# jdhuang-csm/hybrid-drt

Hardware: AMD Instinct MI355X
Metric: DRT fits/sec (256 freq x 512 tau, batched) (higher is better)
Workload: dtype f64

## Files before the change

### hybrid-drt_amd/csrc/gram.hip

```cpp
#include "common.hpp"

namespace hipdrt {

typedef double v4d __attribute__((ext_vector_type(4)));

static constexpr int GT = 64;
static constexpr int GK = 16;
static constexpr int GLD = 80;


template <bool DOP, bool ROWP>
__global__ __launch_bounds__(256, 5) void gram_kernel(int m, int n, const double* __restrict__ A, int lda,
                                                   const double* __restrict__ w, GramL2 g, double* __restrict__ P,
                                                   int ldp, long long p_stride, const int* __restrict__ active,
                                                   int ntile, double* __restrict__ Ppk, long long ppk_stride, int nchp,
                                                   long long a_stride) {
    const int b = blockIdx.y;
    if (active && !active[b]) return;
    A += (size_t)b * a_stride;
    int t = blockIdx.x, ti = 0;
    while (t >= ti + 1) { t -= ti + 1; ++ti; }
    const int tj = t;
    const int i0 = ti * GT, j0 = tj * GT;
    const bool diag = (ti == tj);

    __shared__ double sI[GK * GLD];
    __shared__ double sJ[GK * GLD];

    const int tid = threadIdx.x, lane = tid & 63, wv = tid >> 6;
    const int wi = (wv >> 1) * 32, wj = (wv & 1) * 32;
    const double* wb = w + (size_t)b * m;

    v4d acc[2][2];
#pragma unroll
    for (int a = 0; a < 2; ++a)
#pragma unroll
        for (int c = 0; c < 2; ++c) acc[a][c] = (v4d){0.0, 0.0, 0.0, 0.0};

    const int sk = tid >> 4, sc = (tid & 15) * 4;
    const bool vec2 = ((lda | n) & 1) == 0;
    double vi[4], vj[4], wkr = 0.0;
    auto fetch = [&](int k0) {
        const int k = k0 + sk;
#pragma unroll
        for (int e = 0; e < 4; ++e) { vi[e] = 0.0; vj[e] = 0.0; }
        wkr = 0.0;
        if (k < m) {
            wkr = wb[k];
            const double* row = A + (size_t)k * lda;
            if (vec2) {
#pragma unroll
                for (int e = 0; e < 4; e += 2) {
                    const int ci = i0 + sc + e, cj = j0 + sc + e;
                    if (ci < n) { const double2 t = *reinterpret_cast<const double2*>(row + ci); vi[e] = t.x; vi[e + 1] = t.y; }
                    if (!diag && cj < n) { const double2 t = *reinterpret_cast<const double2*>(row + cj); vj[e] = t.x; vj[e + 1] = t.y; }
                }
            } else {
#pragma unroll
                for (int e = 0; e < 4; ++e) {
                    const int ci = i0 + sc + e, cj = j0 + sc + e;
                    if (ci < n) vi[e] = row[ci];
                    if (!diag && cj < n) vj[e] = row[cj];
                }
            }
        }
    };
    const int nt16 = (n + 15) >> 4;
    const int tr0 = __builtin_amdgcn_readfirstlane((i0 + wi) >> 4), tc0 = __builtin_amdgcn_readfirstlane((j0 + wj) >> 4);
    const bool need00 = tr0 < nt16 && tc0 < nt16 && tr0 >= tc0;
    const bool need01 = tr0 < nt16 && tc0 + 1 < nt16 && tr0 >= tc0 + 1;
    const bool need10 = tr0 + 1 < nt16 && tc0 < nt16 && tr0 + 1 >= tc0;
    const bool need11 = tr0 + 1 < nt16 && tc0 + 1 < nt16 && tr0 + 1 >= tc0 + 1;
    fetch(0);
    for (int k0 = 0; k0 < m; k0 += GK) {
        __syncthreads();
        *reinterpret_cast<double2*>(&sI[sk * GLD + sc]) = make_double2(wkr * vi[0], wkr * vi[1]);
        *reinterpret_cast<double2*>(&sI[sk * GLD + sc + 2]) = make_double2(wkr * vi[2], wkr * vi[3]);
        if (!diag) {
            *reinterpret_cast<double2*>(&sJ[sk * GLD + sc]) = make_double2(wkr * vj[0], wkr * vj[1]);
            *reinterpret_cast<double2*>(&sJ[sk * GLD + sc + 2]) = make_double2(wkr * vj[2], wkr * vj[3]);
        }
        __syncthreads();
        if (k0 + GK < m) fetch(k0 + GK);
        const double* sj = diag ? sI : sJ;
#pragma unroll
        for (int kk = 0; kk < GK; kk += 4) {
            const int kr = kk + (lane >> 4);
            double a0 = sI[kr * GLD + wi + (lane & 15)];
            double a1 = sI[kr * GLD + wi + 16 + (lane & 15)];
            double b0 = sj[kr * GLD + wj + (lane & 15)];
            double b1 = sj[kr * GLD + wj + 16 + (lane & 15)];
            if (need00) acc[0][0] = __builtin_amdgcn_mfma_f64_16x16x4f64(b0, a0, acc[0][0], 0, 0, 0);
            if (need01) acc[0][1] = __builtin_amdgcn_mfma_f64_16x16x4f64(b1, a0, acc[0][1], 0, 0, 0);
            if (need10) acc[1][0] = __builtin_amdgcn_mfma_f64_16x16x4f64(b0, a1, acc[1][0], 0, 0, 0);
            if (need11) acc[1][1] = __builtin_amdgcn_mfma_f64_16x16x4f64(b1, a1, acc[1][1], 0, 0, 0);
        }
    }

    double (*sqI)[GT] = reinterpret_cast<double (*)[GT]>(sI);
    double (*sqJ)[GT] = reinterpret_cast<double (*)[GT]>(sJ);
    constexpr int TW = 2 * GT;
    double (*tw)[TW] = reinterpret_cast<double (*)[TW]>(sI + 3 * GT);
    const int dbase = i0 - j0 - (GT - 1);
    double fac[3] = {0, 0, 0};
    const bool l2on = g.s && !(!DOP && g.toep && g.toep_maxd >= 0 && (j0 >= g.ns || g.spec_zero) && i0 >= g.ns && dbase > g.toep_maxd);
    if (l2on) {
#pragma unroll
        for (int k = 0; k < 3; ++k) fac[k] = g.dfac[k] * (g.use_rho ? g.rho[(size_t)b * 3 + k] : 1.0);
        __syncthreads();
        const double* sb_ = g.s + (size_t)b * 3 * n;
        for (int e = tid; e < 3 * GT; e += 256) {
            const int k = e / GT, c = e % GT;
            sqI[k][c] = (i0 + c < n) ? sqrt(sb_[k * n + i0 + c]) : 0.0;
            sqJ[k][c] = (j0 + c < n) ? sqrt(sb_[k * n + j0 + c]) : 0.0;
        }
        if (g.toep) {
            const int nd = n - g.ns;
            for (int e = tid; e < 3 * TW; e += 256) {
                const int k = e / TW, sl = e % TW;
                int dd = dbase + sl;
                dd = dd < 0 ? -dd : dd;
                tw[k][sl] = (g.dfac[k] > 0.0 && dd < nd) ? g.mk[k][(size_t)g.ns * g.ldm + g.ns + dd] * fac[k] : 0.0;
            }
        }
        __syncthreads();
    }
    double* Pb = (ROWP && P) ? P + (size_t)b * p_stride : nullptr;
    double dfac2[3] = {0, 0, 0};
    if (l2on) {
        if (DOP) {
#pragma unroll
            for (int k = 0; k < 3; ++k) dfac2[k] = g.dop_dfac[k] * (g.use_rho ? g.dop_rho[(size_t)b * 3 + k] : 1.0);
        }
    }
    const int dop_lo = DOP ? g.dop_start : 0, dop_hi = DOP ? g.dop_start + g.dop_size : 0;
    double* Pk = Ppk ? Ppk + (size_t)b * ppk_stride : nullptr;
#pragma unroll
    for (int a = 0; a < 2; ++a)
#pragma unroll
        for (int c = 0; c < 2; ++c) {
            double vals[4];
#pragma unroll
            for (int r = 0; r < 4; ++r) {
                const int i = i0 + wi + a * 16 + (lane & 15);
                const int j = j0 + wj + c * 16 + (lane >> 4) + 4 * r;
                double v = 0.0;
                if (i < n && j < n) {
                    v = acc[a][c][r];
                    if (l2on) {
                        double l2 = 0.0;
#pragma unroll
                        for (int k = 0; k < 3; ++k) {
                            if (g.dfac[k] > 0.0) {
                                double mv;
                                if (g.toep && i >= g.ns && j >= g.ns) {
                                    mv = tw[k][(i - j) - dbase];
                                } else {
                                    mv = g.sym ? g.mk[k][(size_t)j * g.ldm + i] : g.mk[k][(size_t)i * g.ldm + j];
                                    if (i >= g.ns && j >= g.ns) mv *= fac[k];
                                    else if (DOP && i >= dop_lo && i < dop_hi && j >= dop_lo && j < dop_hi) mv *= dfac2[k];
                                }
                                l2 += (sqI[k][i - i0] * mv) * sqJ[k][j - j0];
                            }
                        }
                        v += l2;
                    } else if (!g.s && g.l2) {
                        v += g.l2[(size_t)b * g.l2_stride + (size_t)i * g.ldl2 + j];
                    }
                    if (ROWP && Pb && !(diag && j > i)) {
                        Pb[(size_t)i * ldp + j] = v;
                        if (i != j) Pb[(size_t)j * ldp + i] = v;
                    }
                }
                vals[r] = v;
            }
            if (Pk) {
                const int tr = ((i0 + wi) >> 4) + a, tc = ((j0 + wj) >> 4) + c;
                if (tr < nchp && tc < nchp && tr >= tc) {
                    double2* tile = reinterpret_cast<double2*>(Pk + ((size_t)tr * nchp + tc) * 256);
                    const int fo = (lane & 15) * 4 + (lane >> 4);
                    tile[fo] = make_double2(vals[0], vals[1]);
                    tile[64 + fo] = make_double2(vals[2], vals[3]);
                }
            }
        }
}

__global__ __launch_bounds__(64) void pack_p_kernel(int n, const double* __restrict__ P, int ldp, long long p_stride,
                                                    double* __restrict__ Ppk, long long ppk_stride, int nchp) {
    int t = blockIdx.x, tr = 0;
    while (t >= tr + 1) { t -= tr + 1; ++tr; }
    const int tc = t, b = blockIdx.y, lane = threadIdx.x;
    const double* Pb = P + (size_t)b * p_stride;
    double vals[4];
#pragma unroll
    for (int r = 0; r < 4; ++r) {
        const int i = tr * 16 + (lane & 15), j = tc * 16 + (lane >> 4) + 4 * r;
        double v = 0.0;
        if (i < n && j < n) v = (i >= j) ? Pb[(size_t)i * ldp + j] : Pb[(size_t)j * ldp + i];
        vals[r] = v;
    }
    double2* tile = reinterpret_cast<double2*>(Ppk + (size_t)b * ppk_stride + ((size_t)tr * nchp + tc) * 256);
    const int fo = (lane & 15) * 4 + (lane >> 4);
    tile[fo] = make_double2(vals[0], vals[1]);
    tile[64 + fo] = make_double2(vals[2], vals[3]);
}

__global__ __launch_bounds__(256) void qvec_kernel(int m, int n, const double* __restrict__ A, int lda,
                                                   const double* __restrict__ w, const double* __restrict__ y,
                                                   const double* __restrict__ l1, double l1_scalar,
                                                   double* __restrict__ q, const int* __restrict__ active,
                                                   long long a_stride) {
    const int b = blockIdx.y;
    if (active && !active[b]) return;
    A += (size_t)b * a_stride;
    __shared__ double sw[256], swy[256];
    const int i = blockIdx.x * 256 + threadIdx.x;
    const double* wb = w + (size_t)b * m;
    const double* yb = y + (size_t)b * m;
    double acc = 0.0;
    for (int k0 = 0; k0 < m; k0 += 256) {
        __syncthreads();
        const int kk = k0 + threadIdx.x;
        if (kk < m) { const double wk = wb[kk]; sw[threadIdx.x] = wk; swy[threadIdx.x] = wk * yb[kk]; }
        __syncthreads();
        const int lim = (m - k0) < 256 ? (m - k0) : 256;
        if (i < n) {
            for (int k = 0; k < lim; ++k) acc += (sw[k] * A[(size_t)(k0 + k) * lda + i]) * swy[k];
        }
    }
    if (i < n) q[(size_t)b * n + i] = -acc + (l1 ? l1[i] : l1_scalar);
}

__global__ __launch_bounds__(64) void pack_rows_kernel(int nrow, int ncol, int col_offset, const double* __restrict__ M,
                                                       int ldm, double* __restrict__ tiles, int nchp) {
    const int tr = blockIdx.y, tc = blockIdx.x, lane = threadIdx.x;
    double vals[4];
#pragma unroll
    for (int r = 0; r < 4; ++r) {
        const int i = tr * 16 + (lane & 15), j = tc * 16 + (lane >> 4) + 4 * r - col_offset;
        vals[r] = (i < nrow && j >= 0 && j < ncol) ? M[(size_t)i * ldm + j] : 0.0;
    }
    double2* tile = reinterpret_cast<double2*>(tiles + ((size_t)tr * nchp + tc) * 256);
    const int fo = (lane & 15) * 4 + (lane >> 4);
    tile[fo] = make_double2(vals[0], vals[1]);
    tile[64 + fo] = make_double2(vals[2], vals[3]);
}

void launch_pack_rows(hipStream_t st, int nrow, int ncol, int col_offset, const double* M, int ldm, int ntile_rows,
                      double* tiles, int nchp) {
    hipLaunchKernelGGL(pack_rows_kernel, dim3(nchp, ntile_rows), dim3(64), 0, st, nrow, ncol, col_offset, M, ldm, tiles,
                       nchp);
}

__global__ __launch_bounds__(256) void rows_outer_kernel(const double* __restrict__ Y, int nch, int ncol, int nrow, double scale,
                                                         double* __restrict__ out, int ld) {
    const int ti = blockIdx.y, tj = blockIdx.x;
    if (tj > ti) return;
    __shared__ double A[256], Bt[256];
    const int t = threadIdx.x, i = t >> 4, j = t & 15;
    auto at = [](int r, int k) { return 2 * ((k >> 3) * 64 + r * 4 + (k & 3)) + ((k >> 2) & 1); };
    double acc = 0.0;
    for (int c = 0; c < ncol; ++c) {
        A[t] = Y[((size_t)ti * nch + c) * 256 + t];
        Bt[t] = Y[((size_t)tj * nch + c) * 256 + t];
        __syncthreads();
#pragma unroll
        for (int k = 0; k < 16; ++k) acc += A[at(i, k)] * Bt[at(j, k)];
        __syncthreads();
    }
    const int r = ti * 16 + i, cc = tj * 16 + j;
    if (r < nrow && cc < nrow) {
        out[(size_t)r * ld + cc] = acc * scale;
        out[(size_t)cc * ld + r] = acc * scale;
    }
}

void launch_rows_outer(hipStream_t st, const double* Y, int nch, int ncol, int nex, int nrow, double scale, double* out, int ld) {
    hipLaunchKernelGGL(rows_outer_kernel, dim3(nex, nex), dim3(256), 0, st, Y, nch, ncol, nrow, scale, out, ld);
}

void launch_pack_p(hipStream_t st, int B, int n, const double* P, int ldp, long long p_stride, double* Ppk,
                   long long ppk_stride, int nchp) {
    const int nt = (n + 15) / 16;
    hipLaunchKernelGGL(pack_p_kernel, dim3(nt * (nt + 1) / 2, B), dim3(64), 0, st, n, P, ldp, p_stride, Ppk, ppk_stride,
                       nchp);
}

void launch_gram_l2(hipStream_t st, int B, int m, int n, const double* A, int lda, const double* w, const GramL2& g,
                    double* P, int ldp, long long p_stride, const int* active, double* Ppk, long long ppk_stride,
                    int nchp, long long a_stride) {
    const int nt = (n + GT - 1) / GT;
    const int ntile = nt * (nt + 1) / 2;
    const bool dop = g.s && g.dop_size > 0;
#define HIPDRT_GRAM(D, R) hipLaunchKernelGGL((gram_kernel<D, R>), dim3(ntile, B), dim3(256), 0, st, m, n, A, lda, w, g, P, ldp, \
                                             p_stride, active, ntile, Ppk, ppk_stride, nchp, a_stride)
    if (P) { if (dop) HIPDRT_GRAM(true, true); else HIPDRT_GRAM(false, true); }
    else { if (dop) HIPDRT_GRAM(true, false); else HIPDRT_GRAM(false, false); }
#undef HIPDRT_GRAM
}

void launch_qvec(hipStream_t st, int B, int m, int n, const double* A, int lda, const double* w, const double* y,
                 const double* l1, double l1_scalar, double* q, const int* active, long long a_stride) {
    if (a_stride == 0 && (size_t)m * n < ((size_t)1 << 20)) {
        launch_qvec_batched(st, B, m, n, A, lda, w, y, l1, l1_scalar, q, active);
        return;
    }
    hipLaunchKernelGGL(qvec_kernel, dim3((n + 255) / 256, B), dim3(256), 0, st, m, n, A, lda, w, y, l1, l1_scalar, q,
                       active, a_stride);
}

void launch_weighted_gram(hipStream_t st, int B, int m, int n, const double* A, int lda, const double* w,
                          const double* b, const double* l2, long long l2_stride, int ldl2, const double* l1,
                          double* P, int ldp, long long p_stride, double* q, const int* active) {
    GramL2 g{};
    g.l2 = l2; g.l2_stride = l2_stride; g.ldl2 = ldl2; g.s = nullptr;
    launch_gram_l2(st, B, m, n, A, lda, w, g, P, ldp, p_stride, active);
    launch_qvec(st, B, m, n, A, lda, w, b, l1, 0.0, q, active);
}

}
```

Measured before the change: 2649.

## Redistribute diagonal-tile MFMA work across waves and fold trailing 16-strip

Diagonal 64x64 Gram tiles now spread their ten lower-triangle 16x16 subtiles round-robin over the four waves. Before, waves owning upper-triangle blocks sat idle. When the number of 16-column chunks is 1 mod 4, the leftover 16-wide strip is folded into the diagonal tiles instead of getting its own row of 64-wide tiles, which cuts the tile count. The change adds templated per-turn code paths, extra shared-memory staging for the strip and its L2 weights, and explicit zeroing of padded packed tiles, so code size and complexity grow.

Result: faster. 2700 (median of 6 runs) (+1.9%).

```diff
diff --git a/hybrid-drt_amd/csrc/gram.hip b/hybrid-drt_amd/csrc/gram.hip
--- a/hybrid-drt_amd/csrc/gram.hip
+++ b/hybrid-drt_amd/csrc/gram.hip
@@ -1,4 +1,5 @@
 #include "common.hpp"
+#include <type_traits>
 
 namespace hipdrt {
 
@@ -8,6 +9,29 @@
 static constexpr int GK = 16;
 static constexpr int GLD = 80;
 
+
+__host__ __device__ inline bool gram_strip_folds(int n) { const int nt16 = (n + 15) >> 4; return (nt16 & 3) == 1 && nt16 > 1; }
+
+struct GramSub { int r, c; };
+__host__ __device__ constexpr GramSub gram_diag_sub(int e) {
+    const int r = e >= 10 ? 4 : e >= 6 ? 3 : e >= 3 ? 2 : e >= 1 ? 1 : 0;
+    return GramSub{r, e >= 14 ? 4 : e >= 10 ? e - 10 : e - r * (r + 1) / 2};
+}
+
+template <int TURN>
+__device__ __forceinline__ void gram_diag_slab(const double* sl, v4d (&acc)[4], int needm) {
+#pragma unroll
+    for (int kk = 0; kk < GK; kk += 4) {
+        double x[5];
+#pragma unroll
+        for (int c = 0; c < 5; ++c) x[c] = sl[kk * GLD + c * 16];
+#pragma unroll
+        for (int s = 0; s < 4; ++s) {
+            const GramSub sub = gram_diag_sub(TURN + 4 * s);
+            if (needm & (1 << s)) acc[s] = __builtin_amdgcn_mfma_f64_16x16x4f64(x[sub.c], x[sub.r], acc[s], 0, 0, 0);
+        }
+    }
+}
 
 template <bool DOP, bool ROWP>
 __global__ __launch_bounds__(256, 5) void gram_kernel(int m, int n, const double* __restrict__ A, int lda,
@@ -23,24 +47,41 @@
     const int tj = t;
     const int i0 = ti * GT, j0 = tj * GT;
     const bool diag = (ti == tj);
+    const int nt16 = (n + 15) >> 4;
+    const bool strip = diag && gram_strip_folds(n);
+    const int s0 = (nt16 - 1) * 16;
+    const bool last = strip && i0 + GT == s0;
 
     __shared__ double sI[GK * GLD];
     __shared__ double sJ[GK * GLD];
 
-    const int tid = threadIdx.x, lane = tid & 63, wv = tid >> 6;
-    const int wi = (wv >> 1) * 32, wj = (wv & 1) * 32;
+    const int tid = threadIdx.x, lane = tid & 63, wv = __builtin_amdgcn_readfirstlane(tid >> 6);
     const double* wb = w + (size_t)b * m;
-
-    v4d acc[2][2];
-#pragma unroll
-    for (int a = 0; a < 2; ++a)
-#pragma unroll
-        for (int c = 0; c < 2; ++c) acc[a][c] = (v4d){0.0, 0.0, 0.0, 0.0};
+    double* Pk = Ppk ? Ppk + (size_t)b * ppk_stride : nullptr;
+
+    int nown = 0, needm = 0;
+    const int turn = (wv + 2 * (ti & 1)) & 3;
+    if (diag) {
+        const int rows_all = (Pk && nchp > nt16 ? nchp : nt16) - 4 * ti, rows_data = nt16 - 4 * ti;
+        const int nr = rows_all < 4 ? rows_all : 4, nd = rows_data < 4 ? rows_data : 4;
+        nown = nr * (nr + 1) / 2 + (strip ? 4 : 0) + (last ? 1 : 0);
+        const int nneed = strip ? nown : nd * (nd + 1) / 2;
+#pragma unroll
+        for (int s = 0; s < 4; ++s) needm |= (turn + 4 * s < nneed) << s;
+    }
+    const int qr = 4 * ti + 2 * (wv >> 1), qc = 4 * tj + 2 * (wv & 1);
+    const bool need00 = qr < nt16 && qc < nt16, need01 = qr < nt16 && qc + 1 < nt16;
+    const bool need10 = qr + 1 < nt16 && qc < nt16, need11 = qr + 1 < nt16 && qc + 1 < nt16;
+
+    v4d acc[4];
+#pragma unroll
+    for (int s = 0; s < 4; ++s) acc[s] = (v4d){0.0, 0.0, 0.0, 0.0};
 
     const int sk = tid >> 4, sc = (tid & 15) * 4;
     const bool vec2 = ((lda | n) & 1) == 0;
     double vi[4], vj[4], wkr = 0.0;
-    auto fetch = [&](int k0) {
+    auto fetch = [&](auto DIAG, int k0) {
+        constexpr bool D = decltype(DIAG)::value;
         const int k = k0 + sk;
 #pragma unroll
         for (int e = 0; e < 4; ++e) { vi[e] = 0.0; vj[e] = 0.0; }
@@ -53,57 +94,73 @@
                 for (int e = 0; e < 4; e += 2) {
                     const int ci = i0 + sc + e, cj = j0 + sc + e;
                     if (ci < n) { const double2 t = *reinterpret_cast<const double2*>(row + ci); vi[e] = t.x; vi[e + 1] = t.y; }
-                    if (!diag && cj < n) { const double2 t = *reinterpret_cast<const double2*>(row + cj); vj[e] = t.x; vj[e + 1] = t.y; }
+                    if (!D && cj < n) { const double2 t = *reinterpret_cast<const double2*>(row + cj); vj[e] = t.x; vj[e + 1] = t.y; }
                 }
             } else {
 #pragma unroll
                 for (int e = 0; e < 4; ++e) {
                     const int ci = i0 + sc + e, cj = j0 + sc + e;
                     if (ci < n) vi[e] = row[ci];
-                    if (!diag && cj < n) vj[e] = row[cj];
+                    if (!D && cj < n) vj[e] = row[cj];
                 }
             }
+            if (D && strip && s0 + (tid & 15) < n) vj[0] = row[s0 + (tid & 15)];
         }
     };
-    const int nt16 = (n + 15) >> 4;
-    const int tr0 = __builtin_amdgcn_readfirstlane((i0 + wi) >> 4), tc0 = __builtin_amdgcn_readfirstlane((j0 + wj) >> 4);
-    const bool need00 = tr0 < nt16 && tc0 < nt16 && tr0 >= tc0;
-    const bool need01 = tr0 < nt16 && tc0 + 1 < nt16 && tr0 >= tc0 + 1;
-    const bool need10 = tr0 + 1 < nt16 && tc0 < nt16 && tr0 + 1 >= tc0;
-    const bool need11 = tr0 + 1 < nt16 && tc0 + 1 < nt16 && tr0 + 1 >= tc0 + 1;
-    fetch(0);
-    for (int k0 = 0; k0 < m; k0 += GK) {
-        __syncthreads();
-        *reinterpret_cast<double2*>(&sI[sk * GLD + sc]) = make_double2(wkr * vi[0], wkr * vi[1]);
-        *reinterpret_cast<double2*>(&sI[sk * GLD + sc + 2]) = make_double2(wkr * vi[2], wkr * vi[3]);
-        if (!diag) {
-            *reinterpret_cast<double2*>(&sJ[sk * GLD + sc]) = make_double2(wkr * vj[0], wkr * vj[1]);
-            *reinterpret_cast<double2*>(&sJ[sk * GLD + sc + 2]) = make_double2(wkr * vj[2], wkr * vj[3]);
-        }
-        __syncthreads();
-        if (k0 + GK < m) fetch(k0 + GK);
-        const double* sj = diag ? sI : sJ;
-#pragma unroll
-        for (int kk = 0; kk < GK; kk += 4) {
-            const int kr = kk + (lane >> 4);
-            double a0 = sI[kr * GLD + wi + (lane & 15)];
-            double a1 = sI[kr * GLD + wi + 16 + (lane & 15)];
-            double b0 = sj[kr * GLD + wj + (lane & 15)];
-            double b1 = sj[kr * GLD + wj + 16 + (lane & 15)];
-            if (need00) acc[0][0] = __builtin_amdgcn_mfma_f64_16x16x4f64(b0, a0, acc[0][0], 0, 0, 0);
-            if (need01) acc[0][1] = __builtin_amdgcn_mfma_f64_16x16x4f64(b1, a0, acc[0][1], 0, 0, 0);
-            if (need10) acc[1][0] = __builtin_amdgcn_mfma_f64_16x16x4f64(b0, a1, acc[1][0], 0, 0, 0);
-            if (need11) acc[1][1] = __builtin_amdgcn_mfma_f64_16x16x4f64(b1, a1, acc[1][1], 0, 0, 0);
-        }
-    }
-
-    double (*sqI)[GT] = reinterpret_cast<double (*)[GT]>(sI);
-    double (*sqJ)[GT] = reinterpret_cast<double (*)[GT]>(sJ);
+    auto kloop = [&](auto DIAG, auto TURN) {
+        constexpr bool D = decltype(DIAG)::value;
+        fetch(DIAG, 0);
+        for (int k0 = 0; k0 < m; k0 += GK) {
+            __syncthreads();
+            *reinterpret_cast<double2*>(&sI[sk * GLD + sc]) = make_double2(wkr * vi[0], wkr * vi[1]);
+            *reinterpret_cast<double2*>(&sI[sk * GLD + sc + 2]) = make_double2(wkr * vi[2], wkr * vi[3]);
+            if (!D) {
+                *reinterpret_cast<double2*>(&sJ[sk * GLD + sc]) = make_double2(wkr * vj[0], wkr * vj[1]);
+                *reinterpret_cast<double2*>(&sJ[sk * GLD + sc + 2]) = make_double2(wkr * vj[2], wkr * vj[3]);
+            } else if (strip) {
+                sI[sk * GLD + GT + (tid & 15)] = wkr * vj[0];
+            }
+            __syncthreads();
+            if (k0 + GK < m) fetch(DIAG, k0 + GK);
+            if (!D) {
+                const int wi = (wv >> 1) * 32, wj = (wv & 1) * 32;
+#pragma unroll
+                for (int kk = 0; kk < GK; kk += 4) {
+                    const int kr = kk + (lane >> 4);
+                    double a0 = sI[kr * GLD + wi + (lane & 15)];
+                    double a1 = sI[kr * GLD + wi + 16 + (lane & 15)];
+                    double b0 = sJ[kr * GLD + wj + (lane & 15)];
+                    double b1 = sJ[kr * GLD + wj + 16 + (lane & 15)];
+                    if (need00) acc[0] = __builtin_amdgcn_mfma_f64_16x16x4f64(b0, a0, acc[0], 0, 0, 0);
+                    if (need01) acc[1] = __builtin_amdgcn_mfma_f64_16x16x4f64(b1, a0, acc[1], 0, 0, 0);
+                    if (need10) acc[2] = __builtin_amdgcn_mfma_f64_16x16x4f64(b0, a1, acc[2], 0, 0, 0);
+                    if (need11) acc[3] = __builtin_amdgcn_mfma_f64_16x16x4f64(b1, a1, acc[3], 0, 0, 0);
+                }
+            } else {
+                const double* sl = sI + (lane >> 4) * GLD + (lane & 15);
+                gram_diag_slab<decltype(TURN)::value>(sl, acc, needm);
+            }
+        }
+    };
+    if (!diag) kloop(std::false_type{}, std::integral_constant<int, 0>{});
+    else if (turn == 0) kloop(std::true_type{}, std::integral_constant<int, 0>{});
+    else if (turn == 1) kloop(std::true_type{}, std::integral_constant<int, 1>{});
+    else if (turn == 2) kloop(std::true_type{}, std::integral_constant<int, 2>{});
+    else kloop(std::true_type{}, std::integral_constant<int, 3>{});
+
+    double* sqI = sI;
+    double* sqJ = sJ;
     constexpr int TW = 2 * GT;
-    double (*tw)[TW] = reinterpret_cast<double (*)[TW]>(sI + 3 * GT);
+    double* tw = sI + 3 * GT;
     const int dbase = i0 - j0 - (GT - 1);
+    constexpr int SW = GT + 16;
+    double* sqS = sJ + 3 * GT;
+    double* tws = sJ + 4 * GT;
+    const int dbase_s = s0 - j0 - (GT - 1);
     double fac[3] = {0, 0, 0};
-    const bool l2on = g.s && !(!DOP && g.toep && g.toep_maxd >= 0 && (j0 >= g.ns || g.spec_zero) && i0 >= g.ns && dbase > g.toep_maxd);
+    const bool reach_known = !DOP && g.toep && g.toep_maxd >= 0 && (j0 >= g.ns || g.spec_zero);
+    const bool l2on = g.s && !(reach_known && i0 >= g.ns && dbase > g.toep_maxd);
+    const bool l2on_s = strip && g.s && !(reach_known && s0 >= g.ns && dbase_s > g.toep_maxd);
     if (l2on) {
 #pragma unroll
         for (int k = 0; k < 3; ++k) fac[k] = g.dfac[k] * (g.use_rho ? g.rho[(size_t)b * 3 + k] : 1.0);
@@ -111,8 +168,12 @@
         const double* sb_ = g.s + (size_t)b * 3 * n;
         for (int e = tid; e < 3 * GT; e += 256) {
             const int k = e / GT, c = e % GT;
-            sqI[k][c] = (i0 + c < n) ? sqrt(sb_[k * n + i0 + c]) : 0.0;
-            sqJ[k][c] = (j0 + c < n) ? sqrt(sb_[k * n + j0 + c]) : 0.0;
+            sqI[e] = (i0 + c < n) ? sqrt(sb_[k * n + i0 + c]) : 0.0;
+            sqJ[e] = (j0 + c < n) ? sqrt(sb_[k * n + j0 + c]) : 0.0;
+        }
+        if (strip && tid < 3 * 16) {
+            const int k = tid >> 4, c = tid & 15;
+            sqS[tid] = (s0 + c < n) ? sqrt(sb_[k * n + s0 + c]) : 0.0;
         }
         if (g.toep) {
             const int nd = n - g.ns;
@@ -120,7 +181,11 @@
                 const int k = e / TW, sl = e % TW;
                 int dd = dbase + sl;
                 dd = dd < 0 ? -dd : dd;
-                tw[k][sl] = (g.dfac[k] > 0.0 && dd < nd) ? g.mk[k][(size_t)g.ns * g.ldm + g.ns + dd] * fac[k] : 0.0;
+                tw[e] = (g.dfac[k] > 0.0 && dd < nd) ? g.mk[k][(size_t)g.ns * g.ldm + g.ns + dd] * fac[k] : 0.0;
+            }
+            if (l2on_s && tid < 3 * SW) {
+                const int k = tid / SW, dd = dbase_s + tid % SW;
+                tws[tid] = (g.dfac[k] > 0.0 && dd < nd) ? g.mk[k][(size_t)g.ns * g.ldm + g.ns + dd] * fac[k] : 0.0;
             }
         }
         __syncthreads();
@@ -134,56 +199,81 @@
         }
     }
     const int dop_lo = DOP ? g.dop_start : 0, dop_hi = DOP ? g.dop_start + g.dop_size : 0;
-    double* Pk = Ppk ? Ppk + (size_t)b * ppk_stride : nullptr;
-#pragma unroll
-    for (int a = 0; a < 2; ++a)
-#pragma unroll
-        for (int c = 0; c < 2; ++c) {
-            double vals[4];
-#pragma unroll
-            for (int r = 0; r < 4; ++r) {
-                const int i = i0 + wi + a * 16 + (lane & 15);
-                const int j = j0 + wj + c * 16 + (lane >> 4) + 4 * r;
-                double v = 0.0;
-                if (i < n && j < n) {
-                    v = acc[a][c][r];
-                    if (l2on) {
-                        double l2 = 0.0;
-#pragma unroll
-                        for (int k = 0; k < 3; ++k) {
-                            if (g.dfac[k] > 0.0) {
-                                double mv;
-                                if (g.toep && i >= g.ns && j >= g.ns) {
-                                    mv = tw[k][(i - j) - dbase];
-                                } else {
-                                    mv = g.sym ? g.mk[k][(size_t)j * g.ldm + i] : g.mk[k][(size_t)i * g.ldm + j];
-                                    if (i >= g.ns && j >= g.ns) mv *= fac[k];
-                                    else if (DOP && i >= dop_lo && i < dop_hi && j >= dop_lo && j < dop_hi) mv *= dfac2[k];
-                                }
-                                l2 += (sqI[k][i - i0] * mv) * sqJ[k][j - j0];
+#pragma unroll
+    for (int s = 0; s < 4; ++s) {
+        int r16 = qr + (s >> 1), c16 = qc + (s & 1);
+        bool srow = false, scol = false;
+        if (diag) {
+            const int e = turn + 4 * s;
+            if (e >= nown) continue;
+            const GramSub sub = gram_diag_sub(e);
+            srow = sub.r == 4;
+            scol = sub.c == 4;
+            r16 = srow ? nt16 - 1 : 4 * ti + sub.r;
+            c16 = scol ? nt16 - 1 : 4 * ti + sub.c;
+        }
+        const bool sw = srow && !scol;
+        const bool on = sw ? l2on_s : l2on;
+        const double* sqr = srow ? sqS - s0 : sqI - i0;
+        const double* sqc = scol ? sqS - s0 : sqJ - j0;
+        const int rstr = srow ? 16 : GT, cstr = scol ? 16 : GT;
+        const double* win = sw ? tws - dbase_s : tw - dbase;
+        const int wstr = sw ? SW : TW;
+        double vals[4];
+#pragma unroll
+        for (int r = 0; r < 4; ++r) {
+            const int i = r16 * 16 + (lane & 15);
+            const int j = c16 * 16 + (lane >> 4) + 4 * r;
+            double v = 0.0;
+            if (i < n && j < n) {
+                v = acc[s][r];
+                if (on) {
+                    double l2 = 0.0;
+#pragma unroll
+                    for (int k = 0; k < 3; ++k) {
+                        if (g.dfac[k] > 0.0) {
+                            double mv;
+                            if (g.toep && i >= g.ns && j >= g.ns) {
+                                mv = win[k * wstr + (i - j)];
+                            } else {
+                                mv = g.sym ? g.mk[k][(size_t)j * g.ldm + i] : g.mk[k][(size_t)i * g.ldm + j];
+                                if (i >= g.ns && j >= g.ns) mv *= fac[k];
+                                else if (DOP && i >= dop_lo && i < dop_hi && j >= dop_lo && j < dop_hi) mv *= dfac2[k];
                             }
+                            l2 += (sqr[k * rstr + i] * mv) * sqc[k * cstr + j];
                         }
-                        v += l2;
-                    } else if (!g.s && g.l2) {
-                        v += g.l2[(size_t)b * g.l2_stride + (size_t)i * g.ldl2 + j];
                     }
-                    if (ROWP && Pb && !(diag && j > i)) {
-                        Pb[(size_t)i * ldp + j] = v;
-                        if (i != j) Pb[(size_t)j * ldp + i] = v;
-                    }
+                    v += l2;
+                } else if (!g.s && g.l2) {
+                    v += g.l2[(size_t)b * g.l2_stride + (size_t)i * g.ldl2 + j];
                 }
-                vals[r] = v;
-            }
-            if (Pk) {
-                const int tr = ((i0 + wi) >> 4) + a, tc = ((j0 + wj) >> 4) + c;
-                if (tr < nchp && tc < nchp && tr >= tc) {
-                    double2* tile = reinterpret_cast<double2*>(Pk + ((size_t)tr * nchp + tc) * 256);
-                    const int fo = (lane & 15) * 4 + (lane >> 4);
-                    tile[fo] = make_double2(vals[0], vals[1]);
-                    tile[64 + fo] = make_double2(vals[2], vals[3]);
+                if (ROWP && Pb && j <= i) {
+                    Pb[(size_t)i * ldp + j] = v;
+                    if (i != j) Pb[(size_t)j * ldp + i] = v;
                 }
             }
-        }
+            vals[r] = v;
+        }
+        if (Pk && r16 < nchp && c16 < nchp && r16 >= c16) {
+            double2* tile = reinterpret_cast<double2*>(Pk + ((size_t)r16 * nchp + c16) * 256);
+            const int fo = (lane & 15) * 4 + (lane >> 4);
+            tile[fo] = make_double2(vals[0], vals[1]);
+            tile[64 + fo] = make_double2(vals[2], vals[3]);
+        }
+    }
+    if (Pk && strip) {
+        const int pe = nchp < nt16 + 3 ? nchp : nt16 + 3;
+        for (int pr = nt16; pr < pe; ++pr) {
+#pragma unroll
+            for (int h = 0; h < 2; ++h) {
+                const int pc = h ? nt16 - 1 + wv : 4 * ti + wv;
+                if (h && !(last && pc <= pr)) continue;
+                double2* tile = reinterpret_cast<double2*>(Pk + ((size_t)pr * nchp + pc) * 256);
+                tile[lane] = make_double2(0.0, 0.0);
+                tile[64 + lane] = make_double2(0.0, 0.0);
+            }
+        }
+    }
 }
 
 __global__ __launch_bounds__(64) void pack_p_kernel(int n, const double* __restrict__ P, int ldp, long long p_stride,
@@ -290,7 +380,7 @@
 void launch_gram_l2(hipStream_t st, int B, int m, int n, const double* A, int lda, const double* w, const GramL2& g,
                     double* P, int ldp, long long p_stride, const int* active, double* Ppk, long long ppk_stride,
                     int nchp, long long a_stride) {
-    const int nt = (n + GT - 1) / GT;
+    const int nt = gram_strip_folds(n) ? ((n + 15) / 16) / 4 : (n + GT - 1) / GT;
     const int ntile = nt * (nt + 1) / 2;
     const bool dop = g.s && g.dop_size > 0;
 #define HIPDRT_GRAM(D, R) hipLaunchKernelGGL((gram_kernel<D, R>), dim3(ntile, B), dim3(256), 0, st, m, n, A, lda, w, g, P, ldp, \
```
